# MIT-REALM/gcbfplus

Measured on NVIDIA H100. Metric: env-steps/sec (agents x envs x steps/s) DoubleIntegrator n=512, higher is better.
Workload: dtype f32

## Files before the change

### gcbfplus_b200/csrc/geometry.cu

```cuda
#include <math.h>

#include "common.cuh"
#include "geometry_dev.cuh"

namespace gcbf {

template <int KIND>
__global__ void __launch_bounds__(GB_WARPS * 32)
graph_build_kernel(const gcbf_env_desc d, const float* __restrict__ agent, const float* __restrict__ obstacles,
                   const float* __restrict__ ray_table, float* __restrict__ hits, int32_t* __restrict__ row_start,
                   int32_t* __restrict__ row_deg, int32_t* __restrict__ edge_recv, int32_t* __restrict__ edge_src,
                   int32_t* __restrict__ counters, const int do_cast, const TailArgs tl,
                   float* __restrict__ reward, float* __restrict__ cost, const int rounds) {
    using T = EnvTraits<KIND>;
    constexpr int SD = T::SD, PD = T::PD, NU = T::NU;
    constexpr int OBW = (PD == 2) ? 16 : 4;
    extern __shared__ float smem[];
    const int N = d.n_agents, O = d.n_obs, R = d.n_hits;
    constexpr int OBS2 = (PD == 2) ? OBS2D : 4;
    float* spos = smem;
    float* sobs = spos + N * PD;
    float* stab = sobs + O * OBS2;
    float* salpha = stab + d.n_rays * PD;
    const int n_words = (N + 31) / 32;
    unsigned* sbits = reinterpret_cast<unsigned*>(salpha + (PD == 3 ? GB_WARPS * d.n_rays : 0));
    int* stk = reinterpret_cast<int*>(sbits + GB_WARPS * n_words);
    __shared__ int s_off[GB_WARPS + 1];
    __shared__ int s_base;

    const int g = blockIdx.y;
    const int tid = threadIdx.x, lane = tid & 31, warp = tid >> 5;
    if (O > 0) {
        const float* ob = obstacles + (d.obs_per_graph ? (size_t)g * O * OBW : 0);
        for (int i = tid; i < O * OBW; i += blockDim.x) sobs[(i / OBW) * OBS2 + (i % OBW)] = ob[i];
    }
    for (int i = tid; i < d.n_rays * PD; i += blockDim.x) stab[i] = ray_table[i];
    if (tl.z == nullptr) {
        for (int i = tid; i < N; i += blockDim.x) {
            const float* a = agent + ((size_t)g * N + i) * SD;
#pragma unroll
            for (int c = 0; c < PD; ++c) spos[i * PD + c] = a[c];
        }
    } else {
        __shared__ float s_red[3][GB_WARPS];
        const bool rec = blockIdx.x == 0;
        float acc[3] = {0.f, 0.f, 0.f};
        for (int i = tid; i < N; i += blockDim.x) {
            const size_t a = (size_t)g * N + i;
            float zz[4] = {0.f, 0.f, 0.f, 0.f};
            for (int p = 0; p < tl.parts; ++p) {
                const float4 v = *reinterpret_cast<const float4*>(tl.z + ((size_t)p * tl.z_cap + a) * 4);
                zz[0] += v.x; zz[1] += v.y; zz[2] += v.z; zz[3] += v.w;
            }
            float x[SD], gl[SD], ur[NU], act[NU], xn[SD];
#pragma unroll
            for (int c = 0; c < SD; ++c) {
                x[c] = tl.agent_prev[a * SD + c];
                gl[c] = tl.goal[a * SD + c];
            }
            policy_action<KIND>(d, x, gl, zz, tl.bHO, ur, act);
            if (rec)
#pragma unroll
                for (int c = 0; c < NU; ++c) tl.action[a * NU + c] = act[c];
            const float sq = step_agent<KIND>(d, x, gl, act, ur, true, xn);
#pragma unroll
            for (int c = 0; c < PD; ++c) spos[i * PD + c] = xn[c];
            if (rec) {
#pragma unroll
                for (int c = 0; c < SD; ++c) tl.next_agent[a * SD + c] = xn[c];
                const float nr = sqrtf(sq);
                const bool col = collides_prev<PD, SD>(x, tl.row_start_prev[a], tl.row_deg_prev[a], tl.edge_src_prev,
                                                       tl.agent_prev, d.two_r);
                bool in_obs = false;
                if (O > 0) {
                    const float* ob = obstacles + (d.obs_per_graph ? (size_t)g * O * OBW : 0);
                    in_obs = inside_any<PD>(ob, O, x, d.radius);
                }
                acc[0] += nr * nr;
                acc[1] += col ? 1.f : 0.f;
                acc[2] += in_obs ? 1.f : 0.f;
            }
        }
        if (rec) reduce_reward_cost<GB_WARPS>(acc, &s_red[0][0], N, reward + g, cost + g);
    }
    __syncthreads();
    if (PD == 2) {
        derive_far_fields(sobs, O, d.comm_radius, tid, blockDim.x);
        __syncthreads();
    }

    for (int round = 0; round < rounds; ++round) {
    const int i = (blockIdx.x * rounds + round) * GB_WARPS + warp;
    const bool valid = i < N;
    const int ii = valid ? i : 0;
    float p[PD];
#pragma unroll
    for (int c = 0; c < PD; ++c) p[c] = spos[ii * PD + c];
    const size_t a_glob = (size_t)g * N + ii;
    float* my_hits = hits + a_glob * R * PD;

    if (do_cast && valid) {
        if (PD == 2) {
            lidar2d_warp(p, stab, sobs, O, d.n_rays, R, lane, my_hits);
        } else {
            const bool is_in = (O > 0) ? inside_any<PD>(sobs, O, p, 0.f) : false;
            const float keep = 1.f - (is_in ? 1.f : 0.f);
            float* al = salpha + warp * d.n_rays;
            const float x1 = p[0], y1 = p[1], z1 = p[PD - 1];
            for (int r = lane; r < d.n_rays; r += 32) {
                const float x2 = x1 + stab[r * PD + 0], y2 = y1 + stab[r * PD + 1], z2 = z1 + stab[r * PD + PD - 1];
                float alpha;
                if (O == 0) {
                    alpha = 1.f * NO_HIT;
                } else {
                    alpha = sphere_raytrace(sobs, x1, y1, z1, x2, y2, z2);
                    for (int o = 1; o < O; ++o)
                        alpha = nanmin(alpha, sphere_raytrace(sobs + 4 * o, x1, y1, z1, x2, y2, z2));
                    alpha = alpha * keep;
                }
                al[r] = alpha;
            }
            __syncwarp();
            bool fast = false;
            if (R <= 32) {
                int nA = 0;
                bool odd = false;
                for (int r = lane; r < d.n_rays; r += 32) {
                    const float a = al[r];
                    odd = odd || !(a <= NO_HIT);
                    nA += (a < NO_HIT) ? 1 : 0;
                }
#pragma unroll
                for (int o = 16; o > 0; o >>= 1) nA += __shfl_xor_sync(0xffffffffu, nA, o);
                fast = !__any_sync(0xffffffffu, odd) && nA <= 32 && (d.n_rays - nA) >= R;
                if (fast) {
                    int* tk = stk + warp * 96;
                    const unsigned lt = (1u << lane) - 1u;
                    int nret = 0, nmiss = 0;
                    for (int r0 = 0; r0 < d.n_rays; r0 += 32) {
                        const int r = r0 + lane;
                        const float a = (r < d.n_rays) ? al[r] : NO_HIT;
                        const bool is_ret = (r < d.n_rays) && (a < NO_HIT);
                        const bool is_miss = (r < d.n_rays) && !(a < NO_HIT);
                        const unsigned rb = __ballot_sync(0xffffffffu, is_ret), mb = __ballot_sync(0xffffffffu, is_miss);
                        if (is_ret) {
                            const int pos = nret + __popc(rb & lt);
                            tk[pos] = r;
                            tk[32 + pos] = __float_as_int(a);
                        }
                        if (is_miss) {
                            const int pos = nmiss + __popc(mb & lt);
                            if (pos < 32) tk[64 + pos] = r;
                        }
                        nret += __popc(rb);
                        nmiss += __popc(mb);
                    }
                    __syncwarp();
                    SortKey k;
                    k.flag = (lane < nret) ? 0 : 2;
                    k.alpha = (lane < nret) ? __int_as_float(tk[32 + lane]) : 0.f;
                    k.idx = (lane < nret) ? tk[lane] : (0x40000000 + lane);
                    if (nret > 1) k = warp_sort32(k, lane);
                    if (lane < R) {
                        const int r = (lane < nret) ? k.idx : tk[64 + lane - nret];
                        const float a = (lane < nret) ? k.alpha : NO_HIT;
                        const float x2 = x1 + stab[r * PD + 0], y2 = y1 + stab[r * PD + 1], z2 = z1 + stab[r * PD + PD - 1];
                        my_hits[lane * PD + 0] = x1 + (x2 - x1) * a;
                        my_hits[lane * PD + 1] = y1 + (y2 - y1) * a;
                        my_hits[lane * PD + PD - 1] = z1 + (z2 - z1) * a;
                    }
                }
            }
            for (int rank = 0; rank < (fast ? 0 : R); ++rank) {
                SortKey best;
                best.flag = 3;
                best.alpha = 0.f;
                best.idx = 0x7fffffff;
                for (int r = lane; r < d.n_rays; r += 32) {
                    const float a = al[r];
                    SortKey k;
                    k.flag = (__float_as_uint(a) == 0xffc00001u) ? 3 : (isnan(a) ? 1 : 0);
                    k.alpha = a;
                    k.idx = r;
                    if (key_less(k, best)) best = k;
                }
#pragma unroll
                for (int o = 16; o > 0; o >>= 1) {
                    SortKey other;
                    other.flag = __shfl_xor_sync(0xffffffffu, best.flag, o);
                    other.alpha = __shfl_xor_sync(0xffffffffu, best.alpha, o);
                    other.idx = __shfl_xor_sync(0xffffffffu, best.idx, o);
                    if (key_less(other, best)) best = other;
                }
                if (lane == 0) {
                    const int r = best.idx;
                    const float a = best.alpha;
                    const float x2 = x1 + stab[r * PD + 0], y2 = y1 + stab[r * PD + 1], z2 = z1 + stab[r * PD + PD - 1];
                    my_hits[rank * PD + 0] = x1 + (x2 - x1) * a;
                    my_hits[rank * PD + 1] = y1 + (y2 - y1) * a;
                    my_hits[rank * PD + PD - 1] = z1 + (z2 - z1) * a;
                    al[r] = __uint_as_float(0xffc00001u);
                }
                __syncwarp();
            }
        }
        __syncwarp();
    }
    __syncwarp();

    const unsigned hit_bits = active_hit_bits<PD>(d, p, my_hits, lane, valid);
    int cnt = 0;
    unsigned* my_bits = sbits + warp * n_words;
    if (valid) cnt = neighbour_bits<PD, PD>(d, p, i, spos, lane, my_bits);
    const int deg = valid ? (1 + cnt + __popc(hit_bits)) : 0;
    if (lane == 0) s_off[warp + 1] = deg;
    __syncthreads();
    if (tid == 0) {
        s_off[0] = 0;
        for (int w = 0; w < GB_WARPS; ++w) s_off[w + 1] += s_off[w];
        s_base = (s_off[GB_WARPS] > 0) ? atomicAdd(&counters[0], s_off[GB_WARPS]) : 0;
    }
    __syncthreads();
    const int base = s_base + s_off[warp];
    const int a_id = (int)a_glob;
    if (valid && base + deg > d.edge_cap) {
        if (lane == 0) {
            atomicOr(&counters[1], 1);
            row_start[a_id] = 0;
            row_deg[a_id] = 0;
        }
    } else if (valid) {
        if (lane == 0) {
            row_start[a_id] = base;
            row_deg[a_id] = deg;
        }
        fill_row(edge_recv, edge_src, base, a_id, g * N, my_bits, n_words, hit_bits, lane);
    }
    __syncthreads();
    }
}

constexpr int CANON_T = 512;

__global__ void __launch_bounds__(CANON_T)
edge_canon_stage_kernel(const int A, const int cap, int32_t* __restrict__ row_start, const int32_t* __restrict__ row_deg,
                        const int32_t* __restrict__ edge_src, int32_t* __restrict__ edge_recv) {
    __shared__ int s_warp[CANON_T / 32];
    __shared__ int s_scan[CANON_T];
    __shared__ int s_old[CANON_T];
    const int t = threadIdx.x, lane = t & 31, warp = t >> 5;
    const int a0 = blockIdx.x * CANON_T;
    int pre = 0;
    for (int a = t; a < a0; a += CANON_T) pre += row_deg[a];
#pragma unroll
    for (int o = 16; o > 0; o >>= 1) pre += __shfl_xor_sync(0xffffffffu, pre, o);
    if (lane == 0) s_warp[warp] = pre;
    const int a = a0 + t;
    const int deg = a < A ? row_deg[a] : 0;
    s_old[t] = a < A ? row_start[a] : 0;
    s_scan[t] = deg;
    __syncthreads();
    int base = 0;
    for (int w = 0; w < CANON_T / 32; ++w) base += s_warp[w];
// ... 18 lines not shown
    const int lane = threadIdx.x & 31;
    const int warps = (gridDim.x * blockDim.x) >> 5;
    for (int a = (blockIdx.x * blockDim.x + threadIdx.x) >> 5; a < A; a += warps) {
        const int rs = row_start[a], d = row_deg[a];
        if (rs < 0 || rs + d > cap) continue;
        for (int k = lane; k < d; k += 32) {
            edge_src[rs + k] = edge_recv[rs + k];
            edge_recv[rs + k] = a;
        }
    }
}

template <int KIND>
__global__ void __launch_bounds__(256)
env_step_kernel(const gcbf_env_desc d, const float* __restrict__ agent, const float* __restrict__ goal,
                const float* __restrict__ obstacles, const float* __restrict__ pi,
                const int32_t* __restrict__ row_start, const int32_t* __restrict__ row_deg,
                const int32_t* __restrict__ edge_src, float* __restrict__ action, float* __restrict__ next_agent,
                float* __restrict__ reward, float* __restrict__ cost, const int mode) {
    using T = EnvTraits<KIND>;
    constexpr int SD = T::SD, NU = T::NU, PD = T::PD;
    constexpr int OBW = (PD == 2) ? 16 : 4;
    extern __shared__ float smem[];
    float* sobs = smem;
    __shared__ float red_r[256];
    __shared__ float red_c[256];
    __shared__ float red_o[256];
    const int g = blockIdx.x, N = d.n_agents, O = d.n_obs;
    if (O > 0) {
        const float* ob = obstacles + (d.obs_per_graph ? (size_t)g * O * OBW : 0);
        for (int i = threadIdx.x; i < O * OBW; i += blockDim.x) sobs[i] = ob[i];
    }
    __syncthreads();
    float r_acc = 0.f, c_acc = 0.f, o_acc = 0.f;
    for (int i = threadIdx.x; i < N; i += blockDim.x) {
        const size_t a = (size_t)g * N + i;
        float x[SD], gl[SD], ur[NU], act[NU], xn[SD];
#pragma unroll
        for (int c = 0; c < SD; ++c) {
            x[c] = agent[a * SD + c];
            gl[c] = goal[a * SD + c];
        }
        u_ref_dev<KIND>(d, x, gl, ur);
#pragma unroll
        for (int c = 0; c < NU; ++c) {
            act[c] = (mode == 0) ? (2.f * pi[a * NU + c] + ur[c]) : ((mode == 1 || mode == 3) ? action[a * NU + c] : ur[c]);
            if (mode == 0 || mode == 2) action[a * NU + c] = act[c];
        }
        const float sq = step_agent<KIND>(d, x, gl, act, ur, mode != 3, xn);
#pragma unroll
        for (int c = 0; c < SD; ++c) next_agent[a * SD + c] = xn[c];
        const float nr = sqrtf(sq);
        r_acc += nr * nr;
        const bool col = collides_prev<PD, SD>(x, row_start[a], row_deg[a], edge_src, agent, d.two_r);
        c_acc += col ? 1.f : 0.f;
        o_acc += (O > 0 && inside_any<PD>(sobs, O, x, d.radius)) ? 1.f : 0.f;
    }
    red_r[threadIdx.x] = r_acc;
    red_c[threadIdx.x] = c_acc;
    red_o[threadIdx.x] = o_acc;
    __syncthreads();
    for (int s = 128; s > 0; s >>= 1) {
        if (threadIdx.x < s) {
            red_r[threadIdx.x] += red_r[threadIdx.x + s];
            red_c[threadIdx.x] += red_c[threadIdx.x + s];
            red_o[threadIdx.x] += red_o[threadIdx.x + s];
        }
        __syncthreads();
    }
    if (threadIdx.x == 0) {
        reward[g] = -(red_r[0] / (float)N);
        cost[g] = red_c[0] / (float)N + red_o[0] / (float)N;
    }
}

template <int KIND>
__global__ void __launch_bounds__(GB_WARPS * 32)
masks_kernel(const gcbf_env_desc d, const float* __restrict__ agent, const float* __restrict__ goal,
             const float* __restrict__ hits, const float* __restrict__ obstacles, uint8_t* __restrict__ unsafe,
             uint8_t* __restrict__ collision, uint8_t* __restrict__ finish, uint8_t* __restrict__ safe) {
    using T = EnvTraits<KIND>;
    constexpr int SD = T::SD, PD = T::PD;
    constexpr int OBW = (PD == 2) ? 16 : 4;
    extern __shared__ float smem[];
    const int N = d.n_agents, O = d.n_obs, R = d.n_hits;
    float* spos = smem;
    float* sobs = spos + N * PD;
    const int g = blockIdx.y, tid = threadIdx.x, lane = tid & 31, warp = tid >> 5;
    for (int i = tid; i < N; i += blockDim.x) {
        const float* a = agent + ((size_t)g * N + i) * SD;
#pragma unroll
        for (int c = 0; c < PD; ++c) spos[i * PD + c] = a[c];
    }
    if (O > 0) {
        const float* ob = obstacles + (d.obs_per_graph ? (size_t)g * O * OBW : 0);
        for (int i = tid; i < O * OBW; i += blockDim.x) sobs[i] = ob[i];
    }
    __syncthreads();
    const int i = blockIdx.x * GB_WARPS + warp;
    if (i >= N) return;
    const size_t a = (size_t)g * N + i;
    float x[SD];
#pragma unroll
    for (int c = 0; c < SD; ++c) x[c] = agent[a * SD + c];
    float hx = 0.f, hy = 0.f;
    if (KIND == GCBF_ENV_DOUBLE_INTEGRATOR) {
        const float sp = sqrtf(x[2] * x[2] + x[3] * x[3]);
// ... 475 lines not shown
```

### gcbfplus_b200/csrc/geometry_dev.cuh

```cuda
#pragma once
#include <math.h>

#include "common.cuh"

namespace gcbf {

static constexpr int GB_WARPS = 32;
#define NO_HIT 1e6f

__device__ __forceinline__ bool rect_inside(const float* ob, float px, float py, float r) {
    float rel_x = px - ob[0];
    float rel_y = py - ob[1];
    float rel_xx = fabsf(rel_x * ob[4] + rel_y * ob[5]) - ob[2];
    float rel_yy = fabsf(rel_x * ob[5] - rel_y * ob[4]) - ob[3];
    bool is_in_down = (rel_xx < r) && (rel_yy < 0.f);
    bool is_in_up = (rel_xx < 0.f) && (rel_yy < r);
    bool is_out_corner = (rel_xx > 0.f) && (rel_yy > 0.f);
    bool is_in_circle = sqrtf(rel_xx * rel_xx + rel_yy * rel_yy) < r;
    return (is_in_down || is_in_up) || (is_out_corner && is_in_circle);
}

__device__ __forceinline__ float nanmin(float a, float b) {
    return (isnan(a) || isnan(b)) ? NAN : fminf(a, b);
}
// ... 155 lines not shown
        const float stop = (stop_mask && sqrtf(ddx * ddx + ddy * ddy) < d.half_r) ? 1.f : 0.f;
        const float keep = 1.f - stop;
        xd[0] = (cosf(x[2]) * x[3]) * keep;
        xd[1] = (sinf(x[2]) * x[3]) * keep;
        xd[2] = (u[0] * 20.f) * keep;
        xd[3] = u[1] * keep;
    } else {
#pragma unroll
        for (int r = 0; r < SD; ++r) {
            float s = 0.f;
#pragma unroll
            for (int c = 0; c < SD; ++c) s += x[c] * d.A[r * SD + c];
            float t = 0.f;
#pragma unroll
            for (int c = 0; c < NU; ++c) t += u[c] * d.B[r * NU + c];
            xd[r] = s + t;
        }
    }
#pragma unroll
    for (int c = 0; c < SD; ++c) {
        float v = xd[c] * d.dt + x[c];
        const bool limited = (KIND == GCBF_ENV_DOUBLE_INTEGRATOR && c >= 2) || (KIND == GCBF_ENV_DUBINS_CAR && c == 3) ||
                             (KIND == GCBF_ENV_LINEAR_DRONE && c >= 3);
        if (limited) v = isnan(v) ? v : fminf(fmaxf(v, -d.v_lim), d.v_lim);
        xn[c] = v;
    }
}

template <int KIND>
__device__ __forceinline__ float step_agent(const gcbf_env_desc& d, const float* x, const float* gl, const float* act,
                                            const float* ur, const bool stop_mask, float* xn) {
    constexpr int NU = EnvTraits<KIND>::NU;
    float u[NU], sq = 0.f;
#pragma unroll
    for (int c = 0; c < NU; ++c) {
        u[c] = isnan(act[c]) ? act[c] : fminf(fmaxf(act[c], -d.u_lim), d.u_lim);
        const float df = u[c] - ur[c];
        sq = (c == 0) ? df * df : sq + df * df;
    }
    euler_dev<KIND>(d, x, gl, u, xn, stop_mask);
    return sq;
}

template <int KIND>
__device__ __forceinline__ void policy_action(const gcbf_env_desc& d, const float* x, const float* gl, const float* z,
                                              const float* bHO, float* ur, float* act) {
    u_ref_dev<KIND>(d, x, gl, ur);
#pragma unroll
    for (int c = 0; c < EnvTraits<KIND>::NU; ++c) act[c] = 2.f * tanhf(z[c] + bHO[c]) + ur[c];
}

template <int PD, int SD>
__device__ __forceinline__ bool collides_prev(const float* x, int rs, int rd, const int32_t* edge_src,
                                              const float* agent_prev, float two_r) {
    bool col = false;
    for (int e = rs + 1; e < rs + rd; ++e) {
        const int s = edge_src[e];
        if (s < 0) break;
        float dd = 0.f;
#pragma unroll
        for (int c = 0; c < PD; ++c) {
            const float dlt = x[c] - agent_prev[(size_t)s * SD + c];
            dd = (c == 0) ? dlt * dlt : dd + dlt * dlt;
        }
        col = col || (two_r > sqrtf(dd));
    }
    return col;
}

template <int NW>
__device__ __forceinline__ void reduce_reward_cost(const float* acc, float* s_red, int N, float* reward, float* cost) {
    const int lane = threadIdx.x & 31, warp = threadIdx.x >> 5;
#pragma unroll
    for (int q = 0; q < 3; ++q) {
        const float v = warp_sum(acc[q]);
        if (lane == 0) s_red[q * NW + warp] = v;
    }
    __syncthreads();
    if (threadIdx.x == 0) {
        float t[3] = {0.f, 0.f, 0.f};
        for (int w = 0; w < NW; ++w) {
            t[0] += s_red[0 * NW + w];
            t[1] += s_red[1 * NW + w];
            t[2] += s_red[2 * NW + w];
        }
        *reward = -(t[0] / (float)N);
        *cost = t[1] / (float)N + t[2] / (float)N;
    }
}

constexpr int OBS2D = 24;
__device__ __forceinline__ void derive_far_fields(float* sobs, int O, float comm_radius, int tid, int nthreads) {
    for (int o = tid; o < O; o += nthreads) {
        float* ob = sobs + OBS2D * o;
        const float reach = comm_radius + sqrtf(ob[2] * ob[2] + ob[3] * ob[3]) + 2e-3f;
        ob[14] = reach * reach;
#pragma unroll
        for (int k = 0; k < 4; ++k) {
            const int kp = (k + 3) & 3;
            ob[15 + k] = ob[6 + 2 * kp] - ob[6 + 2 * k];
            ob[19 + k] = ob[7 + 2 * kp] - ob[7 + 2 * k];
        }
    }
}

__device__ __forceinline__ void lidar2d_warp(const float* p, const float* stab, const float* sobs, int O, int n_rays,
                                             int R, int lane, float* my_hits) {
    const bool ray_ok = lane < n_rays;
    const int rl = ray_ok ? lane : 0;
    const float x1 = p[0], y1 = p[1];
    const float x2 = x1 + stab[rl * 2 + 0], y2 = y1 + stab[rl * 2 + 1];
    const float rdx = x1 - x2, rdy = y1 - y2;
    float alpha;
    if (O == 0) {
        alpha = 1.f * NO_HIT;
    } else {
        alpha = NO_HIT;
        bool is_in = false;
        for (int o = 0; o < O; ++o) {
            const float* ob = sobs + OBS2D * o;
            const float cx = x1 - ob[0], cy = y1 - ob[1];
            const bool far = (cx * cx + cy * cy) > ob[14];
            bool degenerate = false;
            if (far) {
#pragma unroll
                for (int k = 0; k < 4; ++k) {
                    const float det = rdx * ob[19 + k] - rdy * ob[15 + k];
                    degenerate = degenerate || !(det != 0.f);
                }
            }
            if (!far) is_in = is_in || rect_inside(ob, x1, y1, 0.f);
            if (!far || __any_sync(0xffffffffu, degenerate))
                alpha = nanmin(alpha, rect_raytrace(ob, x1, y1, x2, y2));
        }
        alpha = alpha * (1.f - (is_in ? 1.f : 0.f));
    }
    const float hx = x1 + (x2 - x1) * alpha;
    const float hy = y1 + (y2 - y1) * alpha;
    SortKey k;
    k.flag = ray_ok ? (isnan(alpha) ? 1 : 0) : 2;
    k.alpha = alpha;
    k.idx = lane;
    const bool all_miss = __all_sync(0xffffffffu, !ray_ok || alpha == NO_HIT);
    if (!all_miss) k = warp_sort32(k, lane);
    const float shx = __shfl_sync(0xffffffffu, hx, k.idx);
    const float shy = __shfl_sync(0xffffffffu, hy, k.idx);
    if (lane < R) {
        my_hits[lane * 2 + 0] = shx;
        my_hits[lane * 2 + 1] = shy;
    }
}

template <int PD>
__device__ __forceinline__ unsigned active_hit_bits(const gcbf_env_desc& d, const float* p, const float* my_hits, int lane,
                                                    bool valid) {
    bool act = false;
    if (valid && lane < d.n_hits) {
        float acc = 0.f;
#pragma unroll
        for (int c = 0; c < PD; ++c) {
            const float dlt = p[c] - my_hits[lane * PD + c];
            acc = (c == 0) ? dlt * dlt : acc + dlt * dlt;
        }
        act = acc < d.lidar_sq_thr;
    }
    return __ballot_sync(0xffffffffu, act);
}

template <int PD, int STRIDE>
__device__ __forceinline__ int neighbour_bits(const gcbf_env_desc& d, const float* p, int i, const float* pos, int lane,
                                              unsigned* my_bits) {
    const int N = d.n_agents;
    int cnt = 0;
    const int n_full = N >> 5;
#pragma unroll 4
    for (int w = 0; w < n_full; ++w) {
        const int j = (w << 5) + lane;
        float acc;
        if (PD == 2) {
            const float2 q = *reinterpret_cast<const float2*>(pos + j * STRIDE);
            const float dx = p[0] - q.x, dy = p[1] - q.y;
            acc = dx * dx;
            acc = acc + dy * dy;
        } else {
            acc = 0.f;
#pragma unroll
            for (int c = 0; c < PD; ++c) {
                const float dlt = p[c] - pos[j * STRIDE + c];
                acc = (c == 0) ? dlt * dlt : acc + dlt * dlt;
            }
        }
        unsigned bits = __ballot_sync(0xffffffffu, acc < d.comm_sq_thr);
        if (w == (i >> 5)) bits &= ~(1u << (i & 31));
        if (lane == 0) my_bits[w] = bits;
        cnt += __popc(bits);
    }
    if (N & 31) {
        const int j = (n_full << 5) + lane;
        bool ok = false;
        if (j < N && j != i) {
            float acc = 0.f;
#pragma unroll
            for (int c = 0; c < PD; ++c) {
                const float dlt = p[c] - pos[j * STRIDE + c];
                acc = (c == 0) ? dlt * dlt : acc + dlt * dlt;
            }
            ok = acc < d.comm_sq_thr;
        }
        const unsigned bits = __ballot_sync(0xffffffffu, ok);
        if (lane == 0) my_bits[n_full] = bits;
        cnt += __popc(bits);
    }
    return cnt;
}
// ... 28 lines not shown
```

### gcbfplus_b200/csrc/rollout_persist.cu

```cuda
#include <stdlib.h>

#include "gemm_tc_prod.cuh"
#include "geometry_dev.cuh"
#include "gnn.cuh"

namespace gcbf {
namespace rp {
using namespace tc;

constexpr int PT = 512;
constexpr int PW = PT / 32;
constexpr int STG = 65536;
constexpr int MAX_N = 512;
constexpr int MAX_OBS = 32;

enum { B_FULL = 0, B_EMPTY = 3, B_B2F = 6, B_B2E = 8, B_MAIN = 10, B_T2F = 11, B_COUNT = 12 };

constexpr int PNU = 2;
enum {
    K_B23 = 0,
    K_BIAS_G = 128,
    K_AVEC = 256,
    K_BU1 = 384,
    K_BU1ROW = 640,
    K_BUH = 896,
    K_HO = 1152,
    K_BHO = K_HO + 256 * PNU,
    K_CST = K_BHO + PNU,
    K_FLOATS = K_CST + 1
};

struct PArgs {
    gcbf_env_desc d;
    int T, cap_env, C;
    const float *W1, *b1, *b23, *bias_g, *avec, *cst, *b_u1, *b_u1row, *buh, *ho, *bho;
    const float *goal, *obstacles, *ray_table;
    float *agent, *hits, *actions, *rewards, *costs;
    int32_t* counters;
    int32_t *row_start, *row_deg, *edge_recv, *edge_src;
    float *msg, *logit, *ag, *v1, *z;
    unsigned long long* prof;
    int soft;
    unsigned* gbar;
};

__device__ __forceinline__ unsigned long long gtime() {
    unsigned long long t;
    asm volatile("mov.u64 %0, %%globaltimer;" : "=l"(t));
    return t;
}
__device__ __forceinline__ void cluster_sync_all() {
    __syncwarp();
    asm volatile("barrier.cluster.arrive.release.aligned;\n\tbarrier.cluster.wait.acquire.aligned;" ::: "memory");
}
__device__ __forceinline__ void soft_group_sync(unsigned* ctr, unsigned target) {
    __syncthreads();
    if (threadIdx.x == 0) {
        __threadfence();
        atomicAdd(ctr, 1u);
        unsigned v;
        const unsigned long long t0 = global_ns();
        do {
            asm volatile("ld.acquire.gpu.global.u32 %0, [%1];" : "=r"(v) : "l"(ctr) : "memory");
            if (v < target && global_ns() - t0 > MBAR_TIMEOUT_NS) __trap();
        } while (v < target);
        __threadfence();
    }
    __syncthreads();
}
__device__ __forceinline__ void fence_async_global() { asm volatile("fence.proxy.async.global;" ::: "memory"); }
template <int KIND>
__global__ void __launch_bounds__(PT, 1)
rollout_persist_kernel(const __grid_constant__ PArgs P, const __grid_constant__ CUtensorMap tmW23h,
                       const __grid_constant__ CUtensorMap tmW23l, const __grid_constant__ CUtensorMap tmA1h,
                       const __grid_constant__ CUtensorMap tmA1l, const __grid_constant__ CUtensorMap tmU1h,
                       const __grid_constant__ CUtensorMap tmU1l, const __grid_constant__ CUtensorMap tmUHh,
                       const __grid_constant__ CUtensorMap tmUHl, const __grid_constant__ CUtensorMap tmAG,
                       const __grid_constant__ CUtensorMap tmV1) {
    using TR = EnvTraits<KIND>;
    constexpr int SD = TR::SD, ED = TR::ED, NU = TR::NU, PD = TR::PD;
    static_assert(PD == 2 && NU == PNU, "persistent rollout kernel: 2-D environments");
    constexpr int OBW = 16, OBS2 = OBS2D;
    constexpr int A_BYTES = 16384, B_BYTES = 16384;
    extern __shared__ uint8_t smem_raw[];
    uint8_t* smem = smem_align1024(smem_raw);
    uint64_t* bars = reinterpret_cast<uint64_t*>(smem + 3 * STG);
    int* s_tot = reinterpret_cast<int*>(smem + 3 * STG + 256 + 16);
    float* sW = reinterpret_cast<float*>(smem + 3 * STG + 512);
    float* sst = sW + 7 * 256;
    float* sobs = sst + MAX_N * 4;
    float* stab = sobs + MAX_OBS * OBS2;
    unsigned* sbits = reinterpret_cast<unsigned*>(stab + 64);
    int* s_off = reinterpret_cast<int*>(sbits + 64 * 16);
// ... 109 lines not shown
                }
            } else if (warp >= 8) {
                const int g = (warp - 8) >> 2, wt = tid & 127;
                const int r = 64 * g + frag_row0(wt);
                const int rs = r + 8 * setup_row(lane);
                uint32_t it_l = it, ne_l = ne;
                for (int tile = lrank; tile < n_tiles; tile += L, ++ne_l) {
                    const int ml = tile * BM + rs;
                    const bool row_ok = ml < M_cur;
                    float fs[ED], f[2][ED];
                    int ss = 0, stype[2];
#pragma unroll
                    for (int c = 0; c < ED; ++c) fs[c] = 0.f;
                    if (row_ok) {
                        const int a = min(max(er_t[seg_e0 + ml], env_a0), env_a0 + N - 1);
                        const int code = min(es_t[seg_e0 + ml], env_a0 + N - 1);
                        float er[ED], es[ED], coef, nrm;
                        edge_state_dev<KIND>(sst + (size_t)(a - env_a0) * SD, er);
                        if (code >= 0) edge_state_dev<KIND>(sst + (size_t)(max(code, env_a0) - env_a0) * SD, es);
                        else sender_state_dev<KIND>(code, a, R, agent_t, P.goal, hits_t, es);
                        edge_feat_dev<KIND>(er, es, code == -1, d.comm_radius, fs, &coef, &nrm);
                        ss = (code >= 0) ? 2 : ((code == -1) ? 1 : 0);
                    }
                    share_rows<ED>(fs, ss, lane, f, stype);
                    const bool ok[2] = {tile * BM + r < M_cur, tile * BM + r + 8 < M_cur};
                    float dacc[64];
                    edge_tile_mainloop<ED>(dacc, smem, &bars[B_FULL], &bars[B_EMPTY], it_l, lane, ok, sW, f, stype);
                    mbar_arrive(&bars[B_MAIN]);
                    bar_consumers();
                    drain_msg(dacc, smem, g, wt, sk + K_B23, P.msg + (seg_e0 + (size_t)tile * BM) * 128, M_cur - tile * BM);
                    fence_async_smem();
                    bar_wg(g);
                    float d2[64];
#pragma unroll
                    for (int i = 0; i < 64; ++i) d2[i] = 0.f;
                    for (int kb2 = 0; kb2 < 4; ++kb2) {
                        const uint32_t j2 = ne_l * 4 + kb2, slot = j2 & 1, use = j2 >> 1;
                        mbar_wait(&bars[B_B2F + slot], use & 1);
                        wg_fence();
                        chain_kblock(d2, smem, g, kb2, slot);
                        wg_commit();
                        wg_wait<0>();
                        mbar_arrive(&bars[B_B2E + slot]);
                    }
                    float q[2][1];
                    frag_relu_dot<1>(d2, sk + K_BIAS_G, sk + K_AVEC, 1, 1, wt, q);
                    if ((lane & 3) == 0) {
                        const int rr = tile * BM + 64 * g + frag_row0(wt);
                        if (rr < M_cur) P.logit[seg_e0 + rr] = q[0][0] + sk[K_CST];
                        if (rr + 8 < M_cur) P.logit[seg_e0 + rr + 8] = q[1][0] + sk[K_CST];
                    }
                    mbar_arrive(&bars[B_T2F]);
                }
            }
            it += 8u * my_tiles;
            ne += my_tiles;
            SYNC_LOCAL();
            if (stamp) pr[1] = gtime();

            for (int il = a_lo + warp; il < a_hi; il += PW) {
                const int a = env_a0 + il;
                const int rs = rs_t[a];
                int rd = rd_t[a];
                if (rs < 0 || rs + rd > cap) rd = 0;
                *reinterpret_cast<float4*>(P.ag + (size_t)a * 128 + lane * 4) =
                    aggregate_logits(rs, rd, P.logit + env_e0, P.msg + env_e0 * 128, lane);
            }
            fence_async_global();
            SYNC_LOCAL();
            if (stamp) pr[2] = gtime();

            const int n_items = ((ga_hi - ga_lo + BM - 1) / BM) * 2;
            const int my_items = (n_items > lrank) ? (n_items - lrank + L - 1) / L : 0;
            float* z_t = P.z + (size_t)(t & 1) * 2 * A_tot * 4;
#pragma unroll 1
            for (int ph2 = 0; ph2 < 2; ++ph2) {
                const int nkb = ph2 == 0 ? 4 : 8;
                const CUtensorMap* tmA = ph2 == 0 ? &tmAG : &tmV1;
                const CUtensorMap* tmBh = ph2 == 0 ? &tmU1h : &tmUHh;
                const CUtensorMap* tmBl = ph2 == 0 ? &tmU1l : &tmUHl;
                if (warp == 0) {
                    if (lane == 0) {
                        uint32_t it_l = it;
                        fence_async_global();
                        for (int item = lrank; item < n_items; item += L) {
                            const int m0 = ga_lo + (item >> 1) * BM, nc0 = (item & 1) * 128;
                            for (int kb = 0; kb < nkb; ++kb, ++it_l) {
                                const int s = it_l % 3;
                                mbar_wait(&bars[B_EMPTY + s], ((it_l / 3) & 1) ^ 1);
                                uint8_t* st = smem + s * STG;
                                mbar_expect_tx(&bars[B_FULL + s], A_BYTES + 2 * B_BYTES);
                                tma_load_2d(st, tmA, &bars[B_FULL + s], kb * BK, env_a0 + m0);
                                tma_load_2d(st + 2 * A_BYTES, tmBh, &bars[B_FULL + s], kb * BK, nc0);
                                tma_load_2d(st + 2 * A_BYTES + B_BYTES, tmBl, &bars[B_FULL + s], kb * BK, nc0);
                            }
                        }
                    }
                } else if (warp >= 8) {
                    const int g = (warp - 8) >> 2, wt = tid & 127;
                    uint32_t it_l = it;
                    for (int item = lrank; item < n_items; item += L) {
                        float dacc[64];
                        tma_a_mainloop(dacc, smem, &bars[B_FULL], &bars[B_EMPTY], it_l, nkb, g, wt);
                        const int m0 = ga_lo + (item >> 1) * BM, nc0 = (item & 1) * 128;
                        const int r0 = m0 + 64 * g + frag_row0(wt);
                        if (ph2 == 0) {
// ... 24 lines not shown
                }
                it += (uint32_t)nkb * my_items;
                if (ph2 == 0) fence_async_global();
                if (ph2 == 0) SYNC_LOCAL();
                else SYNC_ENV((unsigned)t + 1u);
                if (stamp) pr[3 + ph2] = gtime();
            }
        }

        {
            const int tn = t + 1;
            float* agent_n = P.agent + (size_t)tn * A_tot * SD;
            float* hits_n = P.hits + (size_t)tn * A_tot * R * PD;
            const int bn_ = tn & 1;
            int32_t* rs_n = P.row_start + (size_t)bn_ * A_tot;
            int32_t* rd_n = P.row_deg + (size_t)bn_ * A_tot;
            int32_t* er_n = P.edge_recv + (size_t)bn_ * E * cap;
            int32_t* es_n = P.edge_src + (size_t)bn_ * E * cap;
            if (t < 0) {
                for (int i = tid; i < N; i += PT) {
                    const float* a = agent_n + (size_t)(env_a0 + i) * SD;
#pragma unroll
                    for (int c = 0; c < SD; ++c) sst[i * SD + c] = a[c];
                }
            } else {
                const bool rec = rank == 0;
                float acc[3] = {0.f, 0.f, 0.f};
                float* act_t = P.actions + (size_t)t * A_tot * NU;
                for (int i = tid; i < N; i += PT) {
                    const size_t a = (size_t)env_a0 + i;
                    float zz[4] = {0.f, 0.f, 0.f, 0.f};
                    const float* z_t = P.z + (size_t)(t & 1) * 2 * A_tot * 4;
                    for (int p = 0; p < 2; ++p) {
                        const float4 v = *reinterpret_cast<const float4*>(z_t + ((size_t)p * A_tot + a) * 4);
                        zz[0] += v.x; zz[1] += v.y; zz[2] += v.z; zz[3] += v.w;
                    }
                    float x[SD], gl[SD], ur[NU], act[NU], xn[SD];
#pragma unroll
                    for (int c = 0; c < SD; ++c) {
                        x[c] = sst[i * SD + c];
                        gl[c] = P.goal[a * SD + c];
                    }
                    policy_action<KIND>(d, x, gl, zz, sk + K_BHO, ur, act);
                    if (rec)
#pragma unroll
                        for (int c = 0; c < NU; ++c) act_t[a * NU + c] = act[c];
                    const float sq = step_agent<KIND>(d, x, gl, act, ur, true, xn);
#pragma unroll
                    for (int c = 0; c < SD; ++c) sst[i * SD + c] = xn[c];
                    if (rec) {
#pragma unroll
                        for (int c = 0; c < SD; ++c) agent_n[a * SD + c] = xn[c];
                        const float nr = sqrtf(sq);
                        const bool col = collides_prev<PD, SD>(x, rs_t[a], rd_t[a], es_t + env_e0, agent_t, d.two_r);
                        bool in_obs = false;
                        if (O > 0) {
                            const float* ob = P.obstacles + (d.obs_per_graph ? (size_t)env * O * OBW : 0);
                            in_obs = inside_any<PD>(ob, O, x, d.radius);
                        }
                        acc[0] += nr * nr;
                        acc[1] += col ? 1.f : 0.f;
                        acc[2] += in_obs ? 1.f : 0.f;
                    }
                }
                if (rec) reduce_reward_cost<PW>(acc, s_red, N, P.rewards + (size_t)t * E + env, P.costs + (size_t)t * E + env);
            }
            __syncthreads();
            if (stamp) pr[5] = gtime();

            const int n_slots = a_hi - a_lo;
            for (int slot0 = 0; slot0 < APC; slot0 += PW) {
                const int slot = slot0 + warp;
                const int i = a_lo + slot;
                const bool valid = slot < n_slots;
                const int ii = valid ? i : 0;
                float p[PD];
#pragma unroll
                for (int c = 0; c < PD; ++c) p[c] = sst[ii * SD + c];
                const size_t a_glob = (size_t)env_a0 + ii;
                float* my_hits = hits_n + a_glob * R * PD;
                if (valid) lidar2d_warp(p, stab, sobs, O, d.n_rays, R, lane, my_hits);
                __syncwarp();
                const unsigned hit_bits = active_hit_bits<PD>(d, p, my_hits, lane, valid);
                int cnt = 0;
                if (valid) cnt = neighbour_bits<PD, SD>(d, p, i, sst, lane, sbits + slot * n_words);
                if (lane == 0 && slot < APC) {
                    s_off[slot + 1] = valid ? (1 + cnt + __popc(hit_bits)) : 0;
                    s_hb[slot] = hit_bits;
                }
            }
            __syncthreads();
            if (warp == 0) {
                int v0 = (lane < APC) ? s_off[lane + 1] : 0;
                int v1 = (lane + 32 < APC) ? s_off[lane + 33] : 0;
                int inc0 = v0, inc1 = v1;
#pragma unroll
                for (int o = 1; o < 32; o <<= 1) {
                    const int n0_ = __shfl_up_sync(0xffffffffu, inc0, o);
                    const int n1_ = __shfl_up_sync(0xffffffffu, inc1, o);
                    if (lane >= o) { inc0 += n0_; inc1 += n1_; }
                }
                const int tot0 = __shfl_sync(0xffffffffu, inc0, 31);
                __syncwarp();
                if (lane == 0) s_off[0] = 0;
                if (lane < APC) s_off[lane + 1] = inc0;
                if (lane + 32 < APC) s_off[lane + 33] = tot0 + inc1;
                __syncwarp();
                const int total = s_off[APC];
                if (lane < L) {
                    uint32_t ra;
                    asm volatile("mapa.shared::cluster.u32 %0, %1, %2;" : "=r"(ra) : "r"(smem_u32(&s_tot[lrank])), "r"(lane));
                    asm volatile("st.shared::cluster.u32 [%0], %1;" ::"r"(ra), "r"(total) : "memory");
                }
            }
            SYNC_LOCAL();
            if (stamp) pr[6] = gtime();
            int base = 0, env_total = 0;
            for (int r2 = 0; r2 < L; ++r2) {
                const int v = s_tot[r2];
                base += (r2 < lrank) ? v : 0;
                env_total += v;
            }
            for (int slot = warp; slot < n_slots; slot += PW) {
                const int i = a_lo + slot;
                const int a_id = env_a0 + i;
                const int deg = s_off[slot + 1] - s_off[slot];
                const bool over = base + s_off[slot] + deg > seg_cap;
                const int rbase = seg_off + base + s_off[slot];
                if (over) {
                    if (lane == 0) {
                        atomicOr(&P.counters[(size_t)tn * 4 + 1], 1);
                        rs_n[a_id] = 0;
                        rd_n[a_id] = 0;
                    }
                    continue;
                }
                if (lane == 0) {
                    rs_n[a_id] = rbase;
                    rd_n[a_id] = deg;
                }
                fill_row(er_n + env_e0, es_n + env_e0, rbase, a_id, env_a0, sbits + slot * n_words, n_words, s_hb[slot], lane);
            }
            if (lrank == 0 && tid == 0) atomicAdd(&P.counters[(size_t)tn * 4 + 0], min(env_total, seg_cap));
            M_cur = min(env_total, seg_cap);
            SYNC_LOCAL();
            if (stamp) pr[7] = gtime();
        }
    }
#undef SYNC_LOCAL
#undef SYNC_ENV
    if (P.prof != nullptr && rank == 0 && tid == 0) P.prof[(size_t)(P.T + 1) * 8 + 2 * env + 1] = gtime();
}

struct WsLayout {
    int64_t msg, logit, ag, v1, z, row_start, row_deg, edge_recv, edge_src, gbar, total;
};
static WsLayout make_ws_layout(int E, int N, int cap_env) {
    WsLayout W;
    int64_t o = 0;
    auto take = [&](int64_t n) { int64_t r = o; o += (n + 63) & ~(int64_t)63; return r; };
    const int64_t A = (int64_t)E * N, EC = (int64_t)E * cap_env;
    W.msg = take(EC * 128);
    W.logit = take(EC);
    W.ag = take(A * 128 + 128 * 128);
    W.v1 = take(A * 256 + 128 * 256);
    W.z = take(2 * 2 * A * 4);
    W.row_start = take(2 * A);
    W.row_deg = take(2 * A);
    W.edge_recv = take(2 * EC);
    W.edge_src = take(2 * EC);
    W.gbar = take(E);
    W.total = o;
    return W;
}
static int cluster_size(int N, int cap_env) {
    const int items = ((N + 127) / 128) * 2;
    const int tiles = (min(cap_env, 3 * N) + 127) / 128;
    int c = 1;
    while (c < 8 && c < max(items, tiles)) c <<= 1;
    return c;
}

}
}

using namespace gcbf;

extern "C" __attribute__((visibility("default"))) int64_t gcbf_rollout_persistent_workspace_floats(const gcbf_env_desc* desc) {
    if (!desc || desc->edge_cap <= 0 || desc->n_graphs <= 0 || desc->n_agents <= 0) return -1;
    return rp::make_ws_layout(desc->n_graphs, desc->n_agents, desc->edge_cap / desc->n_graphs).total + 64;
}

extern "C" __attribute__((visibility("default"))) int32_t gcbf_rollout_persistent_max_clusters(int32_t cluster_size);

extern "C" __attribute__((visibility("default"))) int32_t gcbf_rollout_persistent_supported(const gcbf_env_desc* desc) {
    if (!desc) return 0;
    const bool ok = desc->env_kind >= 0 && desc->env_kind <= 2 && desc->n_agents >= 1 && desc->n_agents <= rp::MAX_N &&
                    desc->n_obs <= rp::MAX_OBS && desc->n_rays <= 32 && desc->n_hits == desc->n_rays && desc->n_graphs >= 1 &&
                    desc->edge_cap / desc->n_graphs >= desc->n_agents && (desc->obs_per_graph == 1 || desc->n_obs == 0);
    if (!ok) return 0;
    const int C = rp::cluster_size(desc->n_agents, desc->edge_cap / desc->n_graphs);
    static int cached[9] = {0, 0, 0, 0, 0, 0, 0, 0, 0};
    if (cached[C] == 0) {
        const int n = gcbf_rollout_persistent_max_clusters(C);
        cached[C] = n > 0 ? n : -1;
    }
    if (cached[C] > 0 && desc->n_graphs <= cached[C]) return 2;
    if (cached[2] == 0) {
        const int n = gcbf_rollout_persistent_max_clusters(2);
        cached[2] = n > 0 ? n : -1;
    }
    if (C >= 2 && desc->n_graphs * C <= sm_count() && desc->n_graphs * (C / 2) <= cached[2]) return 2;
    return 1;
}

static int persist_smem_bytes() {
    return 3 * rp::STG + 512 + 7 * 256 * 4 + rp::MAX_N * 4 * 4 + rp::MAX_OBS * 24 * 4 + 64 * 4 + 64 * 16 * 4 + 72 * 4 + 64 * 4 +
           3 * rp::PW * 4 + rp::K_FLOATS * 4 + 1024;
}
// ... 32 lines not shown
                     costs && counters && workspace, "gcbf_rollout_persistent: NULL pointer argument");
    GCBF_REQUIRE(gcbf_rollout_persistent_supported(desc) > 0, "gcbf_rollout_persistent: unsupported configuration (2-D envs, "
                 "n_agents <= 512, n_obs <= 32, edge_cap >= n_graphs * n_agents)");
    GCBF_REQUIRE(desc->n_obs == 0 || obstacles, "obstacles is NULL but n_obs > 0");
    GCBF_REQUIRE(n_steps >= 0, "n_steps must be >= 0");
    const int E = desc->n_graphs, N = desc->n_agents;
    const int cap_env = desc->edge_cap / E;
    const rp::WsLayout W = rp::make_ws_layout(E, N, cap_env);
    GCBF_REQUIRE(workspace_floats >= W.total, "workspace too small: %lld < %lld floats", (long long)workspace_floats,
                 (long long)W.total);
    GCBF_REQUIRE(((uintptr_t)workspace & 255) == 0 && ((uintptr_t)actor_params & 15) == 0 && ((uintptr_t)infer_blob & 15) == 0,
                 "workspace must be 256-byte aligned, parameters 16-byte aligned");
    const int ed = env_ed(desc->env_kind), nu = env_nu(desc->env_kind);
    const ParamLayout L = make_layout(ed, nu);
    const InferLayout I = make_infer_layout(nu);
    rp::PArgs P;
    memset(&P, 0, sizeof(P));
    P.d = *desc;
    P.T = n_steps;
    P.cap_env = cap_env;
    P.C = rp::cluster_size(N, cap_env);
    const int max_cl = gcbf_rollout_persistent_max_clusters(P.C);
    static const int force_soft = [] { const char* e = getenv("GCBF_PERSIST_SOFT"); return e ? atoi(e) : -1; }();
    P.soft = (force_soft >= 0) ? (force_soft != 0) : ((E <= max_cl) ? 0 : 1);
    GCBF_REQUIRE(!P.soft || (P.C >= 2 && E * P.C <= sm_count()), "pair mode needs n_graphs * %d <= %d CTAs", P.C, sm_count());
    GCBF_REQUIRE(P.soft || E <= max_cl || force_soft == 0, "more environments (%d) than resident clusters (%d)", E, max_cl);
    P.gbar = reinterpret_cast<unsigned*>(workspace + W.gbar);
    P.W1 = actor_params + L.w[L_MSG0];
    P.b1 = actor_params + L.b[L_MSG0];
    P.b23 = infer_blob + I.b23;
    P.bias_g = actor_params + L.b[L_ATT0];
    P.avec = infer_blob + I.a23;
    P.cst = infer_blob + I.c23;
    P.b_u1 = actor_params + L.b[L_UPD0];
    P.b_u1row = actor_params + L.w[L_UPD0] + 2 * 256;
    P.buh = infer_blob + I.buh;
    P.ho = infer_blob + I.ho;
    P.bho = infer_blob + I.bho;
    P.goal = goal;
    P.obstacles = obstacles;
    P.ray_table = ray_table;
    P.agent = agent_rec;
    P.hits = hits_rec;
    P.actions = actions_rec;
    P.rewards = rewards;
    P.costs = costs;
    P.counters = counters;
    P.prof = reinterpret_cast<unsigned long long*>(phase_stamps);
    P.msg = workspace + W.msg;
    P.logit = workspace + W.logit;
    P.ag = workspace + W.ag;
    P.v1 = workspace + W.v1;
    P.z = workspace + W.z;
    P.row_start = reinterpret_cast<int32_t*>(workspace + W.row_start);
    P.row_deg = reinterpret_cast<int32_t*>(workspace + W.row_deg);
    P.edge_recv = reinterpret_cast<int32_t*>(workspace + W.edge_recv);
    P.edge_src = reinterpret_cast<int32_t*>(workspace + W.edge_src);
    CUtensorMap tW23h, tW23l, tA1h, tA1l, tU1h, tU1l, tUHh, tUHl, tAG, tV1;
    int32_t rc;
#define RC(x) do { if ((rc = (x))) return rc; } while (0)
    RC(tc::make_map(&tW23h, infer_blob + I.t_w23, 128, 256, 128));
    RC(tc::make_map(&tW23l, infer_blob + I.t_w23 + 256 * 128, 128, 256, 128));
    RC(tc::make_map(&tA1h, infer_blob + I.t_a1, 128, 128, 128));
    RC(tc::make_map(&tA1l, infer_blob + I.t_a1 + 128 * 128, 128, 128, 128));
    RC(tc::make_map(&tU1h, infer_blob + I.t_u1, 256, 128, 128));
    RC(tc::make_map(&tU1l, infer_blob + I.t_u1 + 256 * 128, 256, 128, 128));
    RC(tc::make_map(&tUHh, infer_blob + I.t_uh, 256, 256, 128));
    RC(tc::make_map(&tUHl, infer_blob + I.t_uh + 256 * 256, 256, 256, 128));
    RC(tc::make_map(&tAG, P.ag, E * N + 128, 128, 128));
    RC(tc::make_map(&tV1, P.v1, E * N + 128, 256, 128));
#undef RC
    const int smem = persist_smem_bytes();
    cudaLaunchConfig_t cfg;
    memset(&cfg, 0, sizeof(cfg));
    cfg.gridDim = dim3((unsigned)(E * P.C), 1, 1);
    cfg.blockDim = dim3(rp::PT, 1, 1);
    cfg.dynamicSmemBytes = smem;
    cfg.stream = (cudaStream_t)stream;
    cudaLaunchAttribute attr;
    attr.id = cudaLaunchAttributeClusterDimension;
    attr.val.clusterDim.x = (unsigned)(P.soft ? 2 : P.C);
    attr.val.clusterDim.y = 1;
    attr.val.clusterDim.z = 1;
    cfg.attrs = &attr;
    cfg.numAttrs = 1;
    cudaError_t e = cudaSuccess;
    if (P.soft && (e = cudaMemsetAsync(P.gbar, 0, sizeof(unsigned) * E, (cudaStream_t)stream)) != cudaSuccess) {
        set_error("cudaMemsetAsync: %s", cudaGetErrorString(e));
        return (int32_t)e;
    }
    switch (desc->env_kind) {
#define GCBF_RP_CASE(K)                                                                                               \
    case K: {                                                                                                         \
        auto kern = rp::rollout_persist_kernel<K>;                                                                    \
        e = cudaFuncSetAttribute(kern, cudaFuncAttributeMaxDynamicSharedMemorySize, smem);                            \
        if (e == cudaSuccess)                                                                                         \
            e = cudaLaunchKernelEx(&cfg, kern, P, tW23h, tW23l, tA1h, tA1l, tU1h, tU1l, tUHh, tUHl, tAG, tV1);        \
    } break;
        GCBF_RP_CASE(GCBF_ENV_SINGLE_INTEGRATOR)
        GCBF_RP_CASE(GCBF_ENV_DOUBLE_INTEGRATOR)
        GCBF_RP_CASE(GCBF_ENV_DUBINS_CAR)
#undef GCBF_RP_CASE
        default: set_error("gcbf_rollout_persistent: bad env_kind"); return -1;
    }
    if (e != cudaSuccess) {
        set_error("rollout_persist_kernel launch: %s", cudaGetErrorString(e));
// ... 6 lines not shown
```

Measured before the change: 118.2 million.

## Precompute collision/obstacle flags on idle warps and keep lidar hits in registers

Moves the per-agent collision and in-obstacle checks out of the step/reward phase and into otherwise idle warps during the earlier tensor-core phase. They read agent state from shared memory and write flags to a double-buffered workspace array that the reward reduction later reads. Lidar hit coordinates are also returned in registers, so the active-hit test no longer re-reads them from global memory after a warp sync. This adds workspace memory and a cross-phase dependency on the parity-indexed flag buffer.

```diff
diff --git a/gcbfplus_b200/csrc/geometry.cu b/gcbfplus_b200/csrc/geometry.cu
--- a/gcbfplus_b200/csrc/geometry.cu
+++ b/gcbfplus_b200/csrc/geometry.cu
@@ -70,7 +70,7 @@
                 for (int c = 0; c < SD; ++c) tl.next_agent[a * SD + c] = xn[c];
                 const float nr = sqrtf(sq);
                 const bool col = collides_prev<PD, SD>(x, tl.row_start_prev[a], tl.row_deg_prev[a], tl.edge_src_prev,
-                                                       tl.agent_prev, d.two_r);
+                                                       tl.agent_prev, 0, d.two_r);
                 bool in_obs = false;
                 if (O > 0) {
                     const float* ob = obstacles + (d.obs_per_graph ? (size_t)g * O * OBW : 0);
@@ -98,10 +98,15 @@
     for (int c = 0; c < PD; ++c) p[c] = spos[ii * PD + c];
     const size_t a_glob = (size_t)g * N + ii;
     float* my_hits = hits + a_glob * R * PD;
+    float hit[PD];
+    bool hit_in_regs = false;
 
     if (do_cast && valid) {
         if (PD == 2) {
-            lidar2d_warp(p, stab, sobs, O, d.n_rays, R, lane, my_hits);
+            const float2 h = lidar2d_warp(p, stab, sobs, O, d.n_rays, R, lane, my_hits);
+            hit[0] = h.x;
+            hit[PD - 1] = h.y;
+            hit_in_regs = true;
         } else {
             const bool is_in = (O > 0) ? inside_any<PD>(sobs, O, p, 0.f) : false;
             const float keep = 1.f - (is_in ? 1.f : 0.f);
@@ -208,7 +213,10 @@
     }
     __syncwarp();
 
-    const unsigned hit_bits = active_hit_bits<PD>(d, p, my_hits, lane, valid);
+    if (!hit_in_regs && valid && lane < R)
+#pragma unroll
+        for (int c = 0; c < PD; ++c) hit[c] = my_hits[lane * PD + c];
+    const unsigned hit_bits = active_hit_bits<PD>(d, p, hit, lane, valid);
     int cnt = 0;
     unsigned* my_bits = sbits + warp * n_words;
     if (valid) cnt = neighbour_bits<PD, PD>(d, p, i, spos, lane, my_bits);
@@ -333,7 +341,7 @@
         for (int c = 0; c < SD; ++c) next_agent[a * SD + c] = xn[c];
         const float nr = sqrtf(sq);
         r_acc += nr * nr;
-        const bool col = collides_prev<PD, SD>(x, row_start[a], row_deg[a], edge_src, agent, d.two_r);
+        const bool col = collides_prev<PD, SD>(x, row_start[a], row_deg[a], edge_src, agent, 0, d.two_r);
         c_acc += col ? 1.f : 0.f;
         o_acc += (O > 0 && inside_any<PD>(sobs, O, x, d.radius)) ? 1.f : 0.f;
     }
diff --git a/gcbfplus_b200/csrc/geometry_dev.cuh b/gcbfplus_b200/csrc/geometry_dev.cuh
--- a/gcbfplus_b200/csrc/geometry_dev.cuh
+++ b/gcbfplus_b200/csrc/geometry_dev.cuh
@@ -231,7 +231,7 @@
 
 template <int PD, int SD>
 __device__ __forceinline__ bool collides_prev(const float* x, int rs, int rd, const int32_t* edge_src,
-                                              const float* agent_prev, float two_r) {
+                                              const float* agent_prev, int sender0, float two_r) {
     bool col = false;
     for (int e = rs + 1; e < rs + rd; ++e) {
         const int s = edge_src[e];
@@ -239,7 +239,7 @@
         float dd = 0.f;
 #pragma unroll
         for (int c = 0; c < PD; ++c) {
-            const float dlt = x[c] - agent_prev[(size_t)s * SD + c];
+            const float dlt = x[c] - agent_prev[(size_t)(s - sender0) * SD + c];
             dd = (c == 0) ? dlt * dlt : dd + dlt * dlt;
         }
         col = col || (two_r > sqrtf(dd));
@@ -283,8 +283,8 @@
     }
 }
 
-__device__ __forceinline__ void lidar2d_warp(const float* p, const float* stab, const float* sobs, int O, int n_rays,
-                                             int R, int lane, float* my_hits) {
+__device__ __forceinline__ float2 lidar2d_warp(const float* p, const float* stab, const float* sobs, int O, int n_rays,
+                                               int R, int lane, float* my_hits) {
     const bool ray_ok = lane < n_rays;
     const int rl = ray_ok ? lane : 0;
     const float x1 = p[0], y1 = p[1];
@@ -328,17 +328,18 @@
         my_hits[lane * 2 + 0] = shx;
         my_hits[lane * 2 + 1] = shy;
     }
+    return make_float2(shx, shy);
 }
 
 template <int PD>
-__device__ __forceinline__ unsigned active_hit_bits(const gcbf_env_desc& d, const float* p, const float* my_hits, int lane,
+__device__ __forceinline__ unsigned active_hit_bits(const gcbf_env_desc& d, const float* p, const float* hit, int lane,
                                                     bool valid) {
     bool act = false;
     if (valid && lane < d.n_hits) {
         float acc = 0.f;
 #pragma unroll
         for (int c = 0; c < PD; ++c) {
-            const float dlt = p[c] - my_hits[lane * PD + c];
+            const float dlt = p[c] - hit[c];
             acc = (c == 0) ? dlt * dlt : acc + dlt * dlt;
         }
         act = acc < d.lidar_sq_thr;
diff --git a/gcbfplus_b200/csrc/rollout_persist.cu b/gcbfplus_b200/csrc/rollout_persist.cu
--- a/gcbfplus_b200/csrc/rollout_persist.cu
+++ b/gcbfplus_b200/csrc/rollout_persist.cu
@@ -39,6 +39,7 @@
     int32_t* counters;
     int32_t *row_start, *row_deg, *edge_recv, *edge_src;
     float *msg, *logit, *ag, *v1, *z;
+    float2* col_obs;
     unsigned long long* prof;
     int soft;
     unsigned* gbar;
@@ -254,6 +255,21 @@
                     }
                     mbar_arrive(&bars[B_T2F]);
                 }
+            } else {
+                float2* fl = P.col_obs + (size_t)(t & 1) * A_tot;
+                for (int i = a_lo + tid - 32; i < a_hi; i += 7 * 32) {
+                    const size_t a = (size_t)env_a0 + i;
+                    float x[SD];
+#pragma unroll
+                    for (int c = 0; c < SD; ++c) x[c] = sst[i * SD + c];
+                    const bool col = collides_prev<PD, SD>(x, rs_t[a], rd_t[a], es_t + env_e0, sst, env_a0, d.two_r);
+                    bool in_obs = false;
+                    if (O > 0) {
+                        const float* ob = P.obstacles + (d.obs_per_graph ? (size_t)env * O * OBW : 0);
+                        in_obs = inside_any<PD>(ob, O, x, d.radius);
+                    }
+                    fl[a] = make_float2(col ? 1.f : 0.f, in_obs ? 1.f : 0.f);
+                }
             }
             it += 8u * my_tiles;
             ne += my_tiles;
@@ -384,15 +400,10 @@
 #pragma unroll
                         for (int c = 0; c < SD; ++c) agent_n[a * SD + c] = xn[c];
                         const float nr = sqrtf(sq);
-                        const bool col = collides_prev<PD, SD>(x, rs_t[a], rd_t[a], es_t + env_e0, agent_t, d.two_r);
-                        bool in_obs = false;
-                        if (O > 0) {
-                            const float* ob = P.obstacles + (d.obs_per_graph ? (size_t)env * O * OBW : 0);
-                            in_obs = inside_any<PD>(ob, O, x, d.radius);
-                        }
+                        const float2 fl = P.col_obs[(size_t)(t & 1) * A_tot + a];
                         acc[0] += nr * nr;
-                        acc[1] += col ? 1.f : 0.f;
-                        acc[2] += in_obs ? 1.f : 0.f;
+                        acc[1] += fl.x;
+                        acc[2] += fl.y;
                     }
                 }
                 if (rec) reduce_reward_cost<PW>(acc, s_red, N, P.rewards + (size_t)t * E + env, P.costs + (size_t)t * E + env);
@@ -411,9 +422,10 @@
                 for (int c = 0; c < PD; ++c) p[c] = sst[ii * SD + c];
                 const size_t a_glob = (size_t)env_a0 + ii;
                 float* my_hits = hits_n + a_glob * R * PD;
-                if (valid) lidar2d_warp(p, stab, sobs, O, d.n_rays, R, lane, my_hits);
-                __syncwarp();
-                const unsigned hit_bits = active_hit_bits<PD>(d, p, my_hits, lane, valid);
+                float2 h = make_float2(0.f, 0.f);
+                if (valid) h = lidar2d_warp(p, stab, sobs, O, d.n_rays, R, lane, my_hits);
+                const float hit[PD] = {h.x, h.y};
+                const unsigned hit_bits = active_hit_bits<PD>(d, p, hit, lane, valid);
                 int cnt = 0;
                 if (valid) cnt = neighbour_bits<PD, SD>(d, p, i, sst, lane, sbits + slot * n_words);
                 if (lane == 0 && slot < APC) {
@@ -485,7 +497,7 @@
 }
 
 struct WsLayout {
-    int64_t msg, logit, ag, v1, z, row_start, row_deg, edge_recv, edge_src, gbar, total;
+    int64_t msg, logit, ag, v1, z, col_obs, row_start, row_deg, edge_recv, edge_src, gbar, total;
 };
 static WsLayout make_ws_layout(int E, int N, int cap_env) {
     WsLayout W;
@@ -497,6 +509,7 @@
     W.ag = take(A * 128 + 128 * 128);
     W.v1 = take(A * 256 + 128 * 256);
     W.z = take(2 * 2 * A * 4);
+    W.col_obs = take(2 * A * 2);
     W.row_start = take(2 * A);
     W.row_deg = take(2 * A);
     W.edge_recv = take(2 * EC);
@@ -635,6 +648,7 @@
     P.ag = workspace + W.ag;
     P.v1 = workspace + W.v1;
     P.z = workspace + W.z;
+    P.col_obs = reinterpret_cast<float2*>(workspace + W.col_obs);
     P.row_start = reinterpret_cast<int32_t*>(workspace + W.row_start);
     P.row_deg = reinterpret_cast<int32_t*>(workspace + W.row_deg);
     P.edge_recv = reinterpret_cast<int32_t*>(workspace + W.edge_recv);
```

New measurement: 120.6 million, median of 6. +2.0%, better.
